# yangliu9527/Object_SLAM

Measured on AMD Instinct MI355X. Metric: frames/sec tracking+localBA, higher is better.
Workload: dtype f64

## Files before the change

### object_slam_amd/csrc/slam_driver.hip

```cpp
#include <atomic>
#include <chrono>
#include <map>
#include <memory>

#include "common.h"
#include "slam_map.h"
#include "slam_pool.h"

int oslam_slam_make_hip_ops(const oslam_slam_config_t* cfg, oslam_slam_ops_t* out);

namespace oslam_drv {

struct Vocab {
    uint64_t top[10][4], sub[10][10][4];
    Vocab() {
        uint64_t s = 0x853c49e6748fea9bULL;
        auto next = [&]() {
            const uint64_t old = s;
            s = old * 6364136223846793005ULL + 1442695040888963407ULL;
            const uint32_t x = (uint32_t)(((old >> 18u) ^ old) >> 27u), r = (uint32_t)(old >> 59u);
            return (x >> r) | (x << ((-r) & 31));
        };
        auto word = [&]() { const uint64_t hi = next(); const uint64_t lo = next(); return (hi << 32) | lo; };
        for (int i = 0; i < 10; i++)
// ... 237 lines not shown
    k.id = (int)s.map.kfs.size() - 1;
    k.frameId = f.id; k.stamp = f.stamp; k.N = f.N;
    if (!s.lazyKeys) k.keys.assign(f.keys.begin(), f.keys.begin() + f.N);
    k.keysUn.assign(f.keysUn.begin(), f.keysUn.begin() + f.N);
    k.oct.resize(f.N);
    for (int i = 0; i < f.N; i++) k.oct[i] = (uint8_t)f.keysUn[i].octave;
    if (!s.lazyDesc) k.desc.assign(f.desc.begin(), f.desc.begin() + (size_t)f.N * 32);
    k.uRight.assign(f.uRight.begin(), f.uRight.begin() + f.N);
    k.depth.assign(f.depth.begin(), f.depth.begin() + f.N);
    k.mp.assign(f.mp.begin(), f.mp.begin() + f.N);
    k.bowNode = f.bowNode;
    k.pose.set_keyframe(f.pose.Tcw);
    k.Tcp = eye4();
    s.counter.resize(s.map.kfs.size() + 8, 0);
    s.st[1]++;
    s.pendingKF.push_back(k.id);
    s.map.jr_new_kf(k.id);
    return k.id;
}

struct MpUpdate {
    struct Item { int seq, p; };
    std::vector<Item> items;
    std::vector<int> start;
    std::vector<uint8_t> odesc, outdesc;
    std::vector<int32_t> okey;
    std::vector<float> oOw, pos, owref, lsf, out5;
    std::vector<int> best;
    void clear() { items.clear(); }
    void add(int seq, int p) { items.push_back({seq, p}); }
    std::vector<int> dstart;
    std::vector<int32_t> ikey;
    struct Prof {
        std::atomic<long long> ns[4], calls{0}, pts{0}, obs{0};
        Prof() { for (auto& x : ns) x = 0; }
        ~Prof() {
            if (calls.load()) fprintf(stderr, "[mp_update prof] %lld calls, %lld points, %lld observations: count %.1f ms, pack %.1f ms, operator %.1f ms, scatter %.1f ms\n", calls.load(), pts.load(),
                                      obs.load(), ns[0] * 1e-6, ns[1] * 1e-6, ns[2] * 1e-6, ns[3] * 1e-6);
        }
    };
    static Prof* prof() { static Prof* p = getenv("OSLAM_MPU_PROF") ? new Prof : nullptr; static struct D { ~D() { delete prof(); } } d; return p; }
    bool pending = false, pDesc = false, pNormal = false;
    oslam_job_mp_update_t pjob;
    int run(Ctx& c, bool do_desc, bool do_normal) {
        const int rc = submit(c, do_desc, do_normal, false);
        return rc ? rc : finish(c);
    }
    int submit(Ctx& c, bool do_desc, bool do_normal, bool defer) {
        if (pending) { const int rc0 = finish(c); if (rc0) return rc0; }
        const int P = (int)items.size();
        if (P == 0) return OSLAM_OK;
        Prof* pf = prof();
        auto t0_ = std::chrono::steady_clock::now();
        auto lap_ = [&](int k) { if (pf) { auto t1_ = std::chrono::steady_clock::now(); pf->ns[k] += std::chrono::duration_cast<std::chrono::nanoseconds>(t1_ - t0_).count(); t0_ = t1_; } };
        start.assign(P + 1, 0); dstart.assign(P + 1, 0);
        const int chunk = 256, nchunks = (P + chunk - 1) / chunk;
        c.pool->parallel_for(nchunks, [&](int ch) {
            const int i0 = ch * chunk, i1 = std::min(P, i0 + chunk);
            for (int i = i0; i < i1; i++) {
                if (i + kPF < i1) prefetch_mp(&c.seq[items[i + kPF].seq]->map.mps[items[i + kPF].p]);
                if (i + kPF / 2 < i1) __builtin_prefetch(c.seq[items[i + kPF / 2].seq]->map.mps[items[i + kPF / 2].p].obs.data());
                const Map& m = c.seq[items[i].seq]->map;
                const MapPt& p = m.mps[items[i].p];
                int n = 0, nd = 0;
                if (!m.pBad[items[i].p]) { n = (int)p.obs.size(); for (auto& e : p.obs) nd += !m.kfs[e.first].bad; }
                start[i + 1] = n; dstart[i + 1] = nd;
            }
        });
        for (int i = 0; i < P; i++) { start[i + 1] += start[i]; dstart[i + 1] += dstart[i]; }
        lap_(0);
        const size_t total = (size_t)start[P], dtotal = (size_t)dstart[P];
        const bool split = dtotal != total;
        if (do_desc) c.badKFObs.fetch_add((long long)(total - dtotal), std::memory_order_relaxed);
        const bool keyed = c.ops.mp_update_keyed != nullptr && do_desc;
        if (!keyed) odesc.resize(do_desc ? std::max<size_t>(dtotal, 1) * 32 : 32);
        else okey.resize(std::max<size_t>(dtotal, 1) * 3);
        oOw.resize(std::max<size_t>(total, 1) * 3);
        pos.resize((size_t)P * 3); owref.resize((size_t)P * 3); lsf.resize(P);
        c.pool->parallel_for(nchunks, [&](int ch) {
            const int i0 = ch * chunk, i1 = std::min(P, i0 + chunk);
            for (int i = i0; i < i1; i++) {
                if (i + kPF < i1) prefetch_mp(&c.seq[items[i + kPF].seq]->map.mps[items[i + kPF].p]);
                if (i + kPF / 2 < i1) __builtin_prefetch(c.seq[items[i + kPF / 2].seq]->map.mps[items[i + kPF / 2].p].obs.data());
                if (do_normal && i + kPF / 2 < i1) __builtin_prefetch(c.seq[items[i + kPF / 2].seq]->map.mps[items[i + kPF / 2].p].okp.data());
                const Map& m = c.seq[items[i].seq]->map;
                const MapPt& p = m.mps[items[i].p];
                const int n = start[i + 1] - start[i];
                size_t at = (size_t)start[i], dat = (size_t)dstart[i];
                if (n > 0)
                    for (auto& e : p.obs) {
                        const KeyFrm& k = m.kfs[e.first];
                        if (do_desc && !k.bad) {
                            if (keyed) { okey[dat * 3] = items[i].seq; okey[dat * 3 + 1] = e.first; okey[dat * 3 + 2] = e.second; }
                            else memcpy(&odesc[dat * 32], &k.desc[(size_t)e.second * 32], 32);
                            dat++;
                        }
                        oOw[at * 3] = k.pose.Ow[0]; oOw[at * 3 + 1] = k.pose.Ow[1]; oOw[at * 3 + 2] = k.pose.Ow[2];
                        at++;
                    }
                for (int d = 0; d < 3; d++) pos[(size_t)i * 3 + d] = p.pos[d];
                float lf = 1.f;
                const float* ow = p.pos;
                if (n > 0 && p.refKF >= 0) {
                    const KeyFrm& rk = m.kfs[p.refKF];
                    ow = rk.pose.Ow;
                    for (size_t oi = 0; oi < p.obs.size(); oi++)
                        if (p.obs[oi].first == p.refKF) { lf = c.scale[p.okp[oi].octave]; break; }
                }
                for (int d = 0; d < 3; d++) owref[(size_t)i * 3 + d] = ow[d];
                lsf[i] = lf;
            }
        });
        lap_(1);
        best.resize(P); outdesc.resize((size_t)P * 32); out5.resize((size_t)P * 5);
        oslam_job_mp_update_t& j = pjob;
        j.P = P; j.obs_start = start.data(); j.obs_desc = keyed ? nullptr : odesc.data(); j.obs_Ow = oOw.data(); j.Pos = pos.data(); j.OwRef = owref.data();
        j.levelScaleFactor = lsf.data(); j.do_desc = do_desc; j.do_normal = do_normal; j.best_idx = best.data(); j.out_desc = outdesc.data(); j.out5 = out5.data();
        j.desc_start = split ? dstart.data() : nullptr;
        ikey.resize((size_t)P * 2);
        for (int i = 0; i < P; i++) { ikey[2 * (size_t)i] = items[i].seq; ikey[2 * (size_t)i + 1] = items[i].p; }
        j.items = ikey.data();
        const bool async = defer && keyed && c.ops.mp_update_keyed_async && c.ops.mp_update_collect;
        const int rc = async ? c.ops.mp_update_keyed_async(c.ops.ctx, &j, okey.data()) : keyed ? c.ops.mp_update_keyed(c.ops.ctx, &j, okey.data()) : c.ops.mp_update(c.ops.ctx, &j);
        if (rc) return rc;
        lap_(2);
        pending = true; pDesc = do_desc; pNormal = do_normal; pAsync = async;
        if (pf) { pf->calls++; pf->pts += P; pf->obs += (long long)total; }
        return OSLAM_OK;
    }
    bool pAsync = false;
    struct SpecStats { std::atomic<long long> upd{0}, changed{0}, changed_in_list{0}; ~SpecStats() { fprintf(stderr, "[fuse spec stats] per-round descriptor updates %lld, changed %lld, changed and in the current keyframe's candidate list %lld\n", upd.load(), changed.load(), changed_in_list.load()); } };
    int finish(Ctx& c) {
        static SpecStats* spec_stats = getenv("OSLAM_SLAM_SPEC_STATS") ? new SpecStats : nullptr;
        static struct SpecAtExit { ~SpecAtExit() { delete spec_stats; } } spec_at_exit;
        if (!pending) return OSLAM_OK;
        pending = false;
        if (pAsync) { const int rc = c.ops.mp_update_collect(c.ops.ctx); if (rc) return rc; }
        const bool do_desc = pDesc, do_normal = pNormal;
        const int P = (int)items.size();
        const int chunk = 256, nchunks = (P + chunk - 1) / chunk;
        Prof* pf = prof();
        auto t0_ = std::chrono::steady_clock::now();
        auto lap_ = [&](int k) { if (pf) { auto t1_ = std::chrono::steady_clock::now(); pf->ns[k] += std::chrono::duration_cast<std::chrono::nanoseconds>(t1_ - t0_).count(); t0_ = t1_; } };
        c.pool->parallel_for(nchunks, [&](int ch) {
            const int i0 = ch * chunk, i1 = std::min(P, i0 + chunk);
            for (int i = i0; i < i1; i++) {
                if (start[i + 1] == start[i]) continue;
                MapPt& p = c.seq[items[i].seq]->map.mps[items[i].p];
                if (spec_stats && do_desc && !do_normal && dstart[i + 1] > dstart[i]) {
                    spec_stats->upd++;
                    const Seq& sq = *c.seq[items[i].seq];
                    if (memcmp(p.desc, &outdesc[(size_t)i * 32], 32) != 0) { spec_stats->changed++; if (p.fuseListStamp == sq.curKF + 1) spec_stats->changed_in_list++; }
                }
                if (do_desc && dstart[i + 1] > dstart[i]) memcpy(p.desc, &outdesc[(size_t)i * 32], 32);
                if (do_normal) {
                    const float* o = &out5[(size_t)i * 5];
                    p.normal[0] = o[0]; p.normal[1] = o[1]; p.normal[2] = o[2]; p.maxD = o[3]; p.minD = o[4];
                }
                if (do_desc && do_normal) { p.updVer = p.obsVer; p.updStep = c.mapStep; }
            }
        });
        lap_(3);
        return OSLAM_OK;
    }
};

static void create_stereo_points(Ctx& c, Seq& s, Frame& f, int kf, bool all) {
// ... 2023 lines not shown
    TrackInput in(TrackInput::STEREO, left, gray_stride, on_device, timestamps, objs, mask_stride, Tcw_out, state_out);
    in.right = right;
    return track_checked(h, "oslam_slam_track_stereo_objects", in);
}

static void twc_rows(const M4& Tcw, float* o) {
    for (int r = 0; r < 3; r++) {
        for (int cc = 0; cc < 3; cc++) o[r * 4 + cc] = Tcw.m[cc * 4 + r];
        float s = Tcw.m[r] * Tcw.m[3];
        s += Tcw.m[4 + r] * Tcw.m[7];
        s += Tcw.m[8 + r] * Tcw.m[11];
        o[r * 4 + 3] = (float)((double)s * -1.0);
    }
}

int oslam_slam_trajectory(oslam_slam_t* h, int seq, int cap, double* stamps, float* Twc, int32_t* n_out) {
    if (!h || seq < 0 || seq >= h->c.S || !n_out) { oslam::set_error("oslam_slam_trajectory: bad argument"); return OSLAM_E_INVALID; }
    { const int rc_ = oslam_slam_finish(h); if (rc_) return rc_; }
    const Seq& s = *h->c.seq[seq];
    const Map& m = s.map;
    int n = 0;
    if (m.kfs.empty()) { *n_out = 0; return OSLAM_OK; }
    const M4 Two = m.kfs[0].pose.Twc;
    for (const RelPose& r : s.rel) {
        if (r.lost) continue;
        int k = r.refKF;
        M4 Trw = eye4();
        while (m.kfs[k].bad) { Trw = mul4(Trw, m.kfs[k].Tcp); k = m.kfs[k].parent; }
        Trw = mul4(mul4(Trw, m.kfs[k].pose.Tcw), Two);
        const M4 Tcw = mul4(r.Tcr, Trw);
        if (n < cap) {
            if (stamps) stamps[n] = r.stamp;
            if (Twc) twc_rows(Tcw, Twc + (size_t)n * 12);
        }
        n++;
    }
    *n_out = n;
    if (n > cap) { oslam::set_error("trajectory: cap %d < %d", cap, n); return OSLAM_E_CAPACITY; }
    return OSLAM_OK;
}

int oslam_slam_keyframe_trajectory(oslam_slam_t* h, int seq, int cap, double* stamps, float* Twc, int32_t* n_out) {
    if (!h || seq < 0 || seq >= h->c.S || !n_out) { oslam::set_error("oslam_slam_keyframe_trajectory: bad argument"); return OSLAM_E_INVALID; }
    { const int rc_ = oslam_slam_finish(h); if (rc_) return rc_; }
    const Map& m = h->c.seq[seq]->map;
    int n = 0;
    for (const KeyFrm& k : m.kfs) {
        if (k.bad) continue;
        if (n < cap) {
            if (stamps) stamps[n] = k.stamp;
            if (Twc)
                for (int r = 0; r < 3; r++) {
                    for (int cc = 0; cc < 3; cc++) Twc[(size_t)n * 12 + r * 4 + cc] = k.pose.Rwc[r * 3 + cc];
                    Twc[(size_t)n * 12 + r * 4 + 3] = k.pose.Ow[r];
                }
        }
        n++;
    }
    *n_out = n;
    if (n > cap) { oslam::set_error("keyframe trajectory: cap %d < %d", cap, n); return OSLAM_E_CAPACITY; }
    return OSLAM_OK;
}

int oslam_slam_stats(oslam_slam_t* h, int seq, int64_t out[16]) {
    if (!h || seq < 0 || seq >= h->c.S || !out) { oslam::set_error("oslam_slam_stats: bad argument"); return OSLAM_E_INVALID; }
    Seq& s = *h->c.seq[seq];
    memcpy(out, s.st, sizeof(s.st));
    out[2] = s.map.nKFsInMap; out[4] = s.map.nMPsInMap;
    out[15] = map_violations(s.map);
    return OSLAM_OK;
}

int oslam_slam_kernel_times(oslam_slam_t* h, int enable, double out[OSLAM_SLAM_KT_GROUPS * 3]) {
    if (!h) { oslam::set_error("oslam_slam_kernel_times: bad argument"); return OSLAM_E_INVALID; }
    if (!h->c.ops.kernel_times) { oslam::set_error("oslam_slam_kernel_times: this operator table has no device timing"); return OSLAM_E_INVALID; }
    return h->c.ops.kernel_times(h->c.ops.ctx, enable, out);
}

int oslam_slam_debug_point(oslam_slam_t* h, int seq, int id, uint8_t host[64], uint8_t resident[64], int32_t* bad) {
    if (!h || !host || !resident || !bad || seq < 0 || seq >= h->c.S) { oslam::set_error("oslam_slam_debug_point: bad argument"); return OSLAM_E_INVALID; }
    const Map& m = h->c.seq[seq]->map;
    if (id < 0 || id >= (int)m.mps.size()) { oslam::set_error("oslam_slam_debug_point: no such point"); return OSLAM_E_INVALID; }
    const MapPt& p = m.mps[id];
    static_assert(offsetof(MapPt, desc) == 32 && offsetof(MapPt, minD) == 24, "the first 64 bytes of MapPt are the resident record");
    memcpy(host, &p, 64);
    *bad = m.pBad[id] || p.obs.empty();
    if (!h->c.ops.point_record) { oslam::set_error("oslam_slam_debug_point: the operator table keeps no resident map points"); return OSLAM_E_INVALID; }
    return h->c.ops.point_record(h->c.ops.ctx, seq, id, resident);
}

int oslam_slam_bad_keyframe_observations(oslam_slam_t* h, int64_t* out) {
    if (!h || !out) { oslam::set_error("oslam_slam_bad_keyframe_observations: bad argument"); return OSLAM_E_INVALID; }
    *out = h->c.badKFObs.load();
    return OSLAM_OK;
}

int oslam_slam_local_map_reuse(oslam_slam_t* h, int64_t out[2]) {
    if (!h || !out) { oslam::set_error("oslam_slam_local_map_reuse: bad argument"); return OSLAM_E_INVALID; }
    out[0] = h->c.locReuse.load(); out[1] = h->c.locFrames.load();
    return OSLAM_OK;
}

int oslam_slam_struct_sizes(int32_t out[4]) {
    if (!out) return OSLAM_E_INVALID;
    out[0] = (int32_t)sizeof(oslam_slam_config_t); out[1] = (int32_t)sizeof(oslam_slam_ops_t); out[2] = (int32_t)sizeof(oslam_slam_objects_t); out[3] = (int32_t)sizeof(oslam_map_changes_t);
    return OSLAM_OK;
}

int oslam_slam_stage_cpu_seconds(oslam_slam_t* h, double out[16]) {
    if (!h || !out) { oslam::set_error("oslam_slam_stage_cpu_seconds: bad argument"); return OSLAM_E_INVALID; }
    memcpy(out, h->c.cpu, sizeof(h->c.cpu));
    return OSLAM_OK;
}

int oslam_slam_stage_seconds(oslam_slam_t* h, double out[16]) {
    if (!h || !out) { oslam::set_error("oslam_slam_stage_seconds: bad argument"); return OSLAM_E_INVALID; }
    memcpy(out, h->c.sec, sizeof(h->c.sec));
    return OSLAM_OK;
}

}
```

### object_slam_amd/csrc/slam_map.h

```cpp
#pragma once
#include <algorithm>
#include <cmath>
#include <cstdint>
#include <cstring>
#include <map>
#include <set>
#include <utility>
#include <vector>

#include "../../include/oslam_slam.h"

namespace oslam_drv {

typedef oslam_keypoint_t KP;

struct M4 { float m[16]; };
inline M4 eye4() { M4 r; memset(r.m, 0, sizeof(r.m)); r.m[0] = r.m[5] = r.m[10] = r.m[15] = 1.f; return r; }
inline M4 mul4(const M4& a, const M4& b) {
    M4 r;
    for (int i = 0; i < 4; i++)
        for (int j = 0; j < 4; j++) {
            float s = a.m[i * 4] * b.m[j];
            s += a.m[i * 4 + 1] * b.m[4 + j];
            s += a.m[i * 4 + 2] * b.m[8 + j];
            s += a.m[i * 4 + 3] * b.m[12 + j];
            r.m[i * 4 + j] = s;
        }
    return r;
}
inline float norm3(const float* v) {
    double s = 0;
    for (int k = 0; k < 3; k++) s += (double)v[k] * (double)v[k];
    return (float)std::sqrt(s);
}

struct PoseM {
    M4 Tcw, Twc;
    float Rwc[9], Ow[3];
    bool valid = false;
    void set_frame(const M4& T) {
        Tcw = T; valid = true;
        for (int r = 0; r < 3; r++)
            for (int c = 0; c < 3; c++) Rwc[r * 3 + c] = T.m[c * 4 + r];
        for (int r = 0; r < 3; r++) {
            double s = 0;
            for (int k = 0; k < 3; k++) s += (double)T.m[k * 4 + r] * (double)T.m[k * 4 + 3];
            Ow[r] = (float)(-1.0 * s);
        }
        fill_twc();
    }
    void set_keyframe(const M4& T) {
        Tcw = T; valid = true;
        for (int r = 0; r < 3; r++)
            for (int c = 0; c < 3; c++) Rwc[r * 3 + c] = T.m[c * 4 + r];
        for (int r = 0; r < 3; r++) {
            float s = Rwc[r * 3] * T.m[3];
            s += Rwc[r * 3 + 1] * T.m[7];
            s += Rwc[r * 3 + 2] * T.m[11];
            Ow[r] = (float)((double)s * -1.0);
        }
        fill_twc();
    }
    void fill_twc() {
        Twc = eye4();
        for (int r = 0; r < 3; r++) {
            for (int c = 0; c < 3; c++) Twc.m[r * 4 + c] = Rwc[r * 3 + c];
            Twc.m[r * 4 + 3] = Ow[r];
        }
    }
};

struct Frame {
    int id = -1;
    double stamp = 0;
    int N = 0;
    std::vector<KP> keys, keysUn;
    std::vector<uint8_t> desc;
    std::vector<float> uRight, depth;
    std::vector<int> mp;
    std::vector<uint8_t> outlier;
    std::vector<uint32_t> bowNode;
    PoseM pose;
    int refKF = -1;
    oslam_slam_frame_t view;
    struct Obj2D { int det = -1, track = -1, obj3d = -1; std::vector<int> kps; };
    std::vector<Obj2D> objs;
    std::vector<int> objOfKp;
    void alloc(int cap) {
        keys.resize(cap); keysUn.resize(cap); desc.resize((size_t)cap * 32); uRight.resize(cap); depth.resize(cap);
        mp.assign(cap, -1); outlier.assign(cap, 0);
        view.N = 0; view.keys = keys.data(); view.keysUn = keysUn.data(); view.desc = desc.data(); view.uRight = uRight.data(); view.depth = depth.data();
    }
    void begin(int id_, double stamp_) {
        id = id_; stamp = stamp_; N = view.N;
        std::fill(mp.begin(), mp.end(), -1);
        std::fill(outlier.begin(), outlier.end(), 0);
        bowNode.clear(); pose.valid = false; refKF = -1;
        objs.clear(); objOfKp.assign(N, -1);
    }
};

struct ObsKp { float x, y, ur; int octave; };

struct MapPt {
    float pos[3];
    float normal[3] = {0, 0, 0};
    float minD = 0, maxD = 0;
    uint8_t desc[32];
    int firstKF = 0, firstFrame = 0, refKF = -1;
    std::vector<std::pair<int, int>> obs;
    std::vector<ObsKp> okp;
    int trackRefForFrame = 0;
    int fuseListIdx = 0, fuseListStamp = 0;
    int obsVer = 0, updVer = -1, updStep = -1;
    int obs_index(int kf) const {
        for (size_t i = 0; i < obs.size(); i++) if (obs[i].first == kf) return obs[i].second;
        return -1;
    }
};

constexpr int kPF = 12;
inline void prefetch_mp(const MapPt* p) { __builtin_prefetch(p); __builtin_prefetch((const char*)p + 64); __builtin_prefetch((const char*)p + 128); }
template <class Ids>
inline void prefetch_ahead(const std::vector<MapPt>& mps, const Ids& ids, size_t i, size_t n) {
    if (i + kPF < n) { const int q = ids[i + kPF]; if (q >= 0) prefetch_mp(&mps[q]); }
}
template <class Ids>
inline void prefetch_obs_ahead(const std::vector<MapPt>& mps, const Ids& ids, size_t i, size_t n) {
    prefetch_ahead(mps, ids, i, n);
    if (i + kPF / 2 < n) { const int q = ids[i + kPF / 2]; if (q >= 0) __builtin_prefetch(mps[q].obs.data()); }
}

template <class Ids>
inline void prefetch_okp_ahead(const std::vector<MapPt>& mps, const Ids& ids, size_t i, size_t n) {
    prefetch_obs_ahead(mps, ids, i, n);
    if (i + kPF / 2 < n) { const int q = ids[i + kPF / 2]; if (q >= 0) __builtin_prefetch(mps[q].okp.data()); }
}

struct KeyFrm {
    int id = 0, frameId = 0;
    double stamp = 0;
    int N = 0;
    std::vector<KP> keys, keysUn;
    std::vector<uint8_t> desc, oct;
    std::vector<float> uRight, depth;
    std::vector<int> mp;
    std::vector<uint32_t> bowNode;
    PoseM pose;
    M4 Tcp;
    std::map<int, int> connW;
    std::vector<int> ordered, orderedW;
    int parent = -1;
    std::set<int> children;
    bool firstConnection = true, bad = false;
    int trackRefForFrame = 0, fuseTargetForKF = 0;
};

struct RelPose { M4 Tcr; int refKF; double stamp; bool lost; };

struct Map {
    std::vector<MapPt> mps;
    std::vector<KeyFrm> kfs;
    int nKFsInMap = 0, nMPsInMap = 0;
    int64_t nCulledKF = 0, nCulledMP = 0;

    std::vector<int> pNObs, pVisible, pFound, pLastSeen, pReplaced;
    std::vector<uint8_t> pBad;
    std::vector<uint64_t> pLvl;
    bool lvlOverflow = false;
    void lvl_add(int p, int oct) {
        if ((unsigned)oct >= 8u || ((pLvl[p] >> (8 * oct)) & 0xFFull) == 0xFFull) { lvlOverflow = true; return; }
        pLvl[p] += 1ull << (8 * oct);
    }
    void lvl_sub(int p, int oct) {
        if ((unsigned)oct >= 8u || ((pLvl[p] >> (8 * oct)) & 0xFFull) == 0ull) { lvlOverflow = true; return; }
        pLvl[p] -= 1ull << (8 * oct);
    }
    int lvl_count_le(int p, int oct) const {
        const uint64_t h = oct >= 7 ? pLvl[p] : (pLvl[p] & ((1ull << (8 * (oct + 1))) - 1ull));
        uint64_t s2 = (h & 0x00FF00FF00FF00FFull) + ((h >> 8) & 0x00FF00FF00FF00FFull);
        s2 = (s2 & 0x0000FFFF0000FFFFull) + ((s2 >> 16) & 0x0000FFFF0000FFFFull);
        return (int)((s2 & 0xFFFFFFFFull) + (s2 >> 32));
    }
    enum { JR_KFMP = 1, JR_KFMP_BULK = 2, JR_OKF_SET = 3, JR_OKF_CLR = 4, JR_PT = 5, JR_RESET = 6 };
    bool jrOn = false, jrReset = false;
    std::vector<std::pair<int, int>> jrCells;
    std::vector<uint32_t> jrOkf;
    std::vector<int> jrPts, jrNewKFs;
    std::vector<uint8_t> jrPtMark;
    bool jr_pending() const { return jrReset || !jrCells.empty() || !jrOkf.empty() || !jrPts.empty() || !jrNewKFs.empty(); }
    void jr_kfmp(int kf, int idx, int) { if (jrOn) jrCells.push_back(std::make_pair(kf, idx)); }
    void jr_okf(int op, int kf, int idx, int p) { if (jrOn) { jrOkf.push_back((uint32_t)kf); jrOkf.push_back((uint32_t)idx | (op == JR_OKF_SET ? 0x80000000u : 0u)); jrOkf.push_back((uint32_t)p); } }
    void jr_pt(int p) {
        if (!jrOn) return;
        if (jrPtMark.size() <= (size_t)p) jrPtMark.resize((size_t)p + 1 + jrPtMark.size() / 2, 0);
        if (!jrPtMark[p]) { jrPtMark[p] = 1; jrPts.push_back(p); }
    }
    void jr_new_kf(int kf) { if (jrOn) jrNewKFs.push_back(kf); }
    struct JrScratch { std::vector<oslam_map_new_kf_t> kfs; std::vector<uint32_t> good, pts; std::vector<int32_t> cells; std::vector<uint32_t> events; };
    void journal_changes(int slot, float thDepth, JrScratch& sc, oslam_map_changes_t& ch) {
        ch.slot = slot; ch.reset = jrReset ? 1 : 0; jrReset = false;
        sc.kfs.clear(); sc.good.clear();
        size_t gw = 0;
        for (int kf : jrNewKFs) gw += (kfs[kf].mp.size() + 31) / 32;
        sc.good.resize(gw);
        gw = 0;
        for (int kf : jrNewKFs) {
            const KeyFrm& k = kfs[kf];
            const size_t N = k.mp.size(), nw = (N + 31) / 32;
            for (size_t wI = 0; wI < nw; wI++) {
                uint32_t bits = 0;
                for (size_t i = wI * 32; i < std::min(N, wI * 32 + 32); i++) bits |= (uint32_t)(!(k.depth[i] > thDepth || k.depth[i] < 0)) << (i & 31);
                sc.good[gw + wI] = bits;
            }
            oslam_map_new_kf_t e; e.kf = kf; e.N = (int32_t)N; e.mp = k.mp.data(); e.good = nullptr;
            sc.kfs.push_back(e);
            gw += nw;
        }
        gw = 0;
        for (auto& e : sc.kfs) { e.good = sc.good.data() + gw; gw += ((size_t)e.N + 31) / 32; }
        sc.cells.resize(jrCells.size() * 3);
        for (size_t i = 0; i < jrCells.size(); i++) { sc.cells[3 * i] = jrCells[i].first; sc.cells[3 * i + 1] = jrCells[i].second; sc.cells[3 * i + 2] = kfs[jrCells[i].first].mp[jrCells[i].second]; }
        sc.events.swap(jrOkf);
        sc.pts.resize(jrPts.size() * 5);
        for (size_t i = 0; i < jrPts.size(); i++) {
            const int p = jrPts[i];
            jrPtMark[p] = 0;
            sc.pts[5 * i] = (uint32_t)p; sc.pts[5 * i + 1] = (uint32_t)pNObs[p]; sc.pts[5 * i + 2] = (uint32_t)pBad[p];
            sc.pts[5 * i + 3] = (uint32_t)(pLvl[p] & 0xFFFFFFFFull); sc.pts[5 * i + 4] = (uint32_t)(pLvl[p] >> 32);
        }
        ch.n_new = (int32_t)sc.kfs.size(); ch.new_kfs = sc.kfs.data();
        ch.n_cells = (int32_t)jrCells.size(); ch.cells = sc.cells.data();
        ch.n_events = (int32_t)(sc.events.size() / 3); ch.events = sc.events.data();
        ch.n_points = (int32_t)jrPts.size(); ch.points = sc.pts.data();
        jrNewKFs.clear(); jrCells.clear(); jrOkf.clear(); jrPts.clear();
    }
    void set_kf_mp(int kf, int idx, int p) { kfs[kf].mp[idx] = p; jr_kfmp(kf, idx, p); }

    int new_point(const float x[3], int refKF, int refFrame) {
        MapPt p;
        p.pos[0] = x[0]; p.pos[1] = x[1]; p.pos[2] = x[2];
        memset(p.desc, 0, 32);
        p.firstKF = refKF; p.firstFrame = refFrame; p.refKF = refKF;
        mps.push_back(p);
        pNObs.push_back(0); pVisible.push_back(1); pFound.push_back(1);
        pLastSeen.push_back(0); pReplaced.push_back(-1); pBad.push_back(0); pLvl.push_back(0);
        return (int)mps.size() - 1;
    }
    void add_observation(int p, int kf, int idx) {
        MapPt& m = mps[p];
        size_t at = 0;
        while (at < m.obs.size() && m.obs[at].first < kf) at++;
        if (at < m.obs.size() && m.obs[at].first == kf) return;
        const KeyFrm& k = kfs[kf];
        const ObsKp o = {k.keysUn[idx].x, k.keysUn[idx].y, k.uRight[idx], k.keysUn[idx].octave};
        m.obs.insert(m.obs.begin() + at, std::make_pair(kf, idx));
        m.okp.insert(m.okp.begin() + at, o);
        lvl_add(p, o.octave);
        pNObs[p] += o.ur >= 0 ? 2 : 1;
        m.obsVer++;
        jr_okf(JR_OKF_SET, kf, idx, p); jr_pt(p);
    }
    void set_bad_point(int p) {
        MapPt& m = mps[p];
        if (!pBad[p]) { nMPsInMap--; nCulledMP++; }
        pBad[p] = 1;
        std::vector<std::pair<int, int>> o;
        o.swap(m.obs);
        std::vector<ObsKp>().swap(m.okp);
        pLvl[p] = 0;
        for (auto& e : o) { set_kf_mp(e.first, e.second, -1); jr_okf(JR_OKF_CLR, e.first, e.second, p); }
        jr_pt(p);
    }
    void erase_observation(int p, int kf) {
        MapPt& m = mps[p];
        bool bad = false;
        for (size_t i = 0; i < m.obs.size(); i++)
            if (m.obs[i].first == kf) {
                pNObs[p] -= m.okp[i].ur >= 0 ? 2 : 1;
                jr_okf(JR_OKF_CLR, kf, m.obs[i].second, p);
                m.obs.erase(m.obs.begin() + i);
                lvl_sub(p, m.okp[i].octave);
                m.okp.erase(m.okp.begin() + i);
                m.obsVer++;
                if (m.refKF == kf && !m.obs.empty()) m.refKF = m.obs.front().first;
                if (pNObs[p] <= 2) bad = true;
                jr_pt(p);
                break;
            }
        if (bad) set_bad_point(p);
    }
    bool replace_point(int p, int by) {
        if (p == by) return false;
        MapPt& m = mps[p];
        std::vector<std::pair<int, int>> o;
        o.swap(m.obs);
        std::vector<ObsKp>().swap(m.okp);
        pLvl[p] = 0;
        if (!pBad[p]) { nMPsInMap--; }
        pBad[p] = 1;
        pReplaced[p] = by;
        const int nvisible = pVisible[p], nfound = pFound[p];
        for (auto& e : o) {
            jr_okf(JR_OKF_CLR, e.first, e.second, p);
            if (mps[by].obs_index(e.first) < 0) {
                set_kf_mp(e.first, e.second, by);
                add_observation(by, e.first, e.second);
            } else {
                set_kf_mp(e.first, e.second, -1);
            }
        }
        jr_pt(p);
        pFound[by] += nfound;
        pVisible[by] += nvisible;
        return true;
    }

    void update_best_covisibles(int k) {
        KeyFrm& f = kfs[k];
        static thread_local std::vector<std::pair<int, int>> v;
        v.clear();
        for (auto& e : f.connW) v.push_back(std::make_pair(e.second, e.first));
        std::sort(v.begin(), v.end());
        f.ordered.clear(); f.orderedW.clear();
        for (size_t i = v.size(); i-- > 0;) { f.ordered.push_back(v[i].second); f.orderedW.push_back(v[i].first); }
    }
    void add_connection(int k, int other, int w) {
        KeyFrm& f = kfs[k];
        auto it = f.connW.find(other);
        if (it == f.connW.end()) f.connW[other] = w;
        else if (it->second != w) it->second = w;
        else return;
        update_best_covisibles(k);
    }
    void erase_connection(int k, int other) {
        if (kfs[k].connW.erase(other)) update_best_covisibles(k);
    }
    struct IntSpan {
        const int* b; const int* e;
        const int* begin() const { return b; }
        const int* end() const { return e; }
        size_t size() const { return (size_t)(e - b); }
    };
    IntSpan best_covisibles(int k, int n) const {
        const KeyFrm& f = kfs[k];
        const size_t m = std::min<size_t>(f.ordered.size(), (size_t)std::max(n, 0));
        return IntSpan{f.ordered.data(), f.ordered.data() + m};
    }
    int weight(int k, int other) const {
        auto it = kfs[k].connW.find(other);
        return it == kfs[k].connW.end() ? 0 : it->second;
    }
    void update_connections(int k, std::vector<int>& counter ) {
        KeyFrm& f = kfs[k];
        static thread_local std::vector<int> touched;
        touched.clear();
        for (int i = 0; i < f.N; i++) {
            prefetch_obs_ahead(mps, f.mp, i, f.N);
            const int p = f.mp[i];
            if (p < 0 || pBad[p]) continue;
            for (auto& e : mps[p].obs) {
                if (e.first == k) continue;
                if (counter[e.first]++ == 0) touched.push_back(e.first);
            }
        }
        if (touched.empty()) return;
        std::sort(touched.begin(), touched.end());
        int nmax = 0, kmax = -1;
        const int th = 15;
        static thread_local std::vector<std::pair<int, int>> v2;
        std::vector<std::pair<int, int>>& v = v2;
        v.clear();
        for (int o : touched) {
            const int c = counter[o];
            if (c > nmax) { nmax = c; kmax = o; }
            if (c >= th) { v.push_back(std::make_pair(c, o)); add_connection(o, k, c); }
        }
        if (v.empty()) { v.push_back(std::make_pair(nmax, kmax)); add_connection(kmax, k, nmax); }
        std::sort(v.begin(), v.end());
        f.connW.clear();
        for (int o : touched) { f.connW[o] = counter[o]; counter[o] = 0; }
        f.ordered.clear(); f.orderedW.clear();
        for (size_t i = v.size(); i-- > 0;) { f.ordered.push_back(v[i].second); f.orderedW.push_back(v[i].first); }
        if (f.firstConnection && f.id != 0) {
            f.parent = f.ordered.front();
            kfs[f.parent].children.insert(k);
            f.firstConnection = false;
        }
    }
    int tracked_map_points(int k, int minObs) const {
        const KeyFrm& f = kfs[k];
        int n = 0;
        for (int i = 0; i < f.N; i++) {
            const int p = f.mp[i];
// ... 44 lines not shown
```

Baseline: 46560.

## Move map points and observation lists into a per-sequence slab arena

Map points now live in a chunked table backed by a per-sequence arena built on hugepage-advised mmap slabs. Each point's observation and keypoint lists, which were two std::vectors, become one arena block holding both arrays. MapPt is repacked to 128 bytes with the per-frame fields in the first cache line. The aim is to cut malloc traffic, pointer chasing and TLB misses during tracking and local BA. In exchange it adds custom allocator complexity, and the table can no longer be copied or grown as a contiguous vector.

```diff
diff --git a/object_slam_amd/csrc/seq_arena.h b/object_slam_amd/csrc/seq_arena.h
--- /dev/null
+++ b/object_slam_amd/csrc/seq_arena.h
@@ -0,0 +1,221 @@
+#pragma once
+#include <cstddef>
+#include <cstdint>
+#include <cstdlib>
+#include <cstring>
+#include <mutex>
+#include <new>
+#include <type_traits>
+
+#ifndef OSLAM_ARENA_PASSTHROUGH
+#include <sys/mman.h>
+#endif
+
+#ifndef OSLAM_ARENA_CHUNK_KB
+#define OSLAM_ARENA_CHUNK_KB 16
+#endif
+
+namespace oslam_drv {
+
+constexpr size_t kArenaChunk = (size_t)OSLAM_ARENA_CHUNK_KB << 10;
+constexpr size_t kArenaSlab = (size_t)64 << 20;
+constexpr size_t kArenaHuge = (size_t)2 << 20;
+constexpr size_t kArenaChunkHead = 64;
+
+struct ArenaChunk { ArenaChunk* next; };
+
+struct SlabPoolStats { size_t slabs, chunks_carved, chunks_free, madvise_failed; bool hugepages; };
+
+#ifndef OSLAM_ARENA_PASSTHROUGH
+class SlabPool {
+public:
+    static SlabPool& instance() { static SlabPool p; return p; }
+    ArenaChunk* take() {
+        std::lock_guard<std::mutex> g(mu_);
+        if (free_) { ArenaChunk* c = free_; free_ = c->next; nFree_--; return c; }
+        if (cur_ == end_) {
+            char* raw = (char*)mmap(nullptr, kArenaSlab + kArenaHuge, PROT_READ | PROT_WRITE, MAP_PRIVATE | MAP_ANONYMOUS, -1, 0);
+            if (raw == (char*)MAP_FAILED) throw std::bad_alloc();
+            char* al = (char*)(((uintptr_t)raw + kArenaHuge - 1) & ~(uintptr_t)(kArenaHuge - 1));
+            if (al > raw) munmap(raw, (size_t)(al - raw));
+            if (al + kArenaSlab < raw + kArenaSlab + kArenaHuge) munmap(al + kArenaSlab, (size_t)(raw + kArenaHuge - al));
+            if (huge_ && madvise(al, kArenaSlab, MADV_HUGEPAGE) != 0) nMadvFail_++;
+            cur_ = al; end_ = al + kArenaSlab; nSlabs_++;
+        }
+        ArenaChunk* c = (ArenaChunk*)cur_;
+        cur_ += kArenaChunk; nCarved_++;
+        return c;
+    }
+    void give(ArenaChunk* head, ArenaChunk* tail, size_t n) {
+        std::lock_guard<std::mutex> g(mu_);
+        tail->next = free_; free_ = head; nFree_ += n;
+    }
+    SlabPoolStats stats() {
+        std::lock_guard<std::mutex> g(mu_);
+        return SlabPoolStats{nSlabs_, nCarved_, nFree_, nMadvFail_, huge_};
+    }
+private:
+    SlabPool() { const char* e = getenv("OSLAM_MAP_HUGEPAGES"); huge_ = !(e && e[0] == '0'); }
+    std::mutex mu_;
+    ArenaChunk* free_ = nullptr;
+    char *cur_ = nullptr, *end_ = nullptr;
+    size_t nSlabs_ = 0, nCarved_ = 0, nFree_ = 0, nMadvFail_ = 0;
+    bool huge_ = true;
+};
+#endif
+
+class SeqArena {
+public:
+    static constexpr int kClasses = 24;
+    static size_t class_units(int c) { return c == 0 ? 1 : (c & 1) ? (size_t)1 << ((c + 1) / 2) : (size_t)3 << (c / 2 - 1); }
+    static size_t class_bytes(int c) { return class_units(c) << 4; }
+    static int class_of(size_t bytes) {
+        const size_t u = (bytes + 15) >> 4;
+        if (u <= 1) return 0;
+        const int p = 63 - __builtin_clzll((unsigned long long)u);
+        if (u == (size_t)1 << p) return 2 * p - 1;
+        if (u <= (size_t)3 << (p - 1)) return 2 * p;
+        return 2 * p + 1;
+    }
+    static constexpr size_t kMaxSmall = kArenaChunk / 2;
+
+    SeqArena() = default;
+    SeqArena(const SeqArena&) = delete;
+    SeqArena& operator=(const SeqArena&) = delete;
+    SeqArena(SeqArena&& o) noexcept { steal(o); }
+    SeqArena& operator=(SeqArena&& o) noexcept { if (this != &o) { release(); steal(o); } return *this; }
+    ~SeqArena() { release(); }
+
+    void* alloc(size_t bytes) {
+#ifndef OSLAM_ARENA_PASSTHROUGH
+        if (bytes <= kMaxSmall) {
+            const int c = class_of(bytes);
+            if (free_[c]) { void* p = free_[c]; free_[c] = *(void**)p; return p; }
+            const size_t sz = class_bytes(c);
+            if (void* p = bump(sz)) return p;
+            for (int c2 = c + 1; c2 < kClasses; c2++)
+                if (free_[c2]) {
+                    char* b = (char*)free_[c2]; free_[c2] = *(void**)b;
+                    recycle(b + sz, b + class_bytes(c2));
+                    return b;
+                }
+            if (cur_) recycle(cur_, end_);
+            ArenaChunk* ch = SlabPool::instance().take();
+            ch->next = chunks_; chunks_ = ch; nChunks_++;
+            if (!lastChunk_) lastChunk_ = ch;
+            cur_ = (char*)ch + kArenaChunkHead; end_ = (char*)ch + kArenaChunk;
+            return bump(sz);
+        }
+#endif
+        return tracked_alloc(bytes);
+    }
+    void dealloc(void* p, size_t bytes) {
+        if (!p) return;
+#ifndef OSLAM_ARENA_PASSTHROUGH
+        if (bytes <= kMaxSmall) { const int c = class_of(bytes); *(void**)p = free_[c]; free_[c] = p; return; }
+#endif
+        (void)bytes;
+        tracked_free(p);
+    }
+    void release() {
+        while (big_) tracked_free((char*)big_ + sizeof(Big));
+#ifndef OSLAM_ARENA_PASSTHROUGH
+        if (chunks_) SlabPool::instance().give(chunks_, lastChunk_, nChunks_);
+        chunks_ = lastChunk_ = nullptr; nChunks_ = 0; cur_ = end_ = nullptr;
+        memset(free_, 0, sizeof(free_));
+#endif
+    }
+    size_t chunks_held() const { return nChunks_; }
+
+private:
+    struct alignas(64) Big { Big *prev, *next; };
+    void* tracked_alloc(size_t bytes) {
+        void* raw = nullptr;
+        if (posix_memalign(&raw, 64, sizeof(Big) + bytes) != 0) throw std::bad_alloc();
+        Big* b = (Big*)raw;
+        b->prev = nullptr; b->next = big_;
+        if (big_) big_->prev = b;
+        big_ = b;
+        return (char*)b + sizeof(Big);
+    }
+    void tracked_free(void* p) {
+        Big* b = (Big*)((char*)p - sizeof(Big));
+        if (b->prev) b->prev->next = b->next; else big_ = b->next;
+        if (b->next) b->next->prev = b->prev;
+        free(b);
+    }
+    void steal(SeqArena& o) {
+        big_ = o.big_; o.big_ = nullptr;
+        chunks_ = o.chunks_; lastChunk_ = o.lastChunk_; nChunks_ = o.nChunks_; cur_ = o.cur_; end_ = o.end_;
+        memcpy(free_, o.free_, sizeof(free_));
+        o.chunks_ = o.lastChunk_ = nullptr; o.nChunks_ = 0; o.cur_ = o.end_ = nullptr;
+        memset(o.free_, 0, sizeof(o.free_));
+    }
+#ifndef OSLAM_ARENA_PASSTHROUGH
+    void* bump(size_t sz) {
+        if (!cur_) return nullptr;
+        char* p = cur_;
+        if (sz >= 1024) p = (char*)(((uintptr_t)p + 63) & ~(uintptr_t)63);
+        if (p + sz > end_) return nullptr;
+        if (p != cur_) recycle(cur_, p);
+        cur_ = p + sz;
+        return p;
+    }
+    void recycle(char* b, char* e) {
+        while (e - b >= 16) {
+            size_t rem = (size_t)(e - b);
+            if (rem > kMaxSmall) rem = kMaxSmall;
+            int c = class_of(rem);
+            if (class_bytes(c) > rem) c--;
+            const size_t mis = (uintptr_t)b & 63;
+            if (class_bytes(c) >= 1024 && mis) c = class_of(64 - mis);
+            *(void**)b = free_[c]; free_[c] = b;
+            b += class_bytes(c);
+        }
+    }
+#endif
+    Big* big_ = nullptr;
+    ArenaChunk *chunks_ = nullptr, *lastChunk_ = nullptr;
+    size_t nChunks_ = 0;
+    char *cur_ = nullptr, *end_ = nullptr;
+    void* free_[kClasses] = {};
+};
+
+template <class T, int K>
+struct ChunkVec {
+    static_assert(std::is_trivially_copyable<T>::value && std::is_trivially_destructible<T>::value, "ChunkVec holds plain data");
+    static constexpr size_t kMask = ((size_t)1 << K) - 1;
+    T** blk = nullptr;
+    uint32_t nblk = 0, capblk = 0;
+    size_t n = 0;
+    ChunkVec() = default;
+    ChunkVec(const ChunkVec&) = delete;
+    ChunkVec& operator=(const ChunkVec&) = delete;
+    ChunkVec(ChunkVec&& o) noexcept : blk(o.blk), nblk(o.nblk), capblk(o.capblk), n(o.n) { o.blk = nullptr; o.nblk = o.capblk = 0; o.n = 0; }
+    ChunkVec& operator=(ChunkVec&& o) noexcept {
+        if (this != &o) { blk = o.blk; nblk = o.nblk; capblk = o.capblk; n = o.n; o.blk = nullptr; o.nblk = o.capblk = 0; o.n = 0; }
+        return *this;
+    }
+    T& operator[](size_t i) { return blk[i >> K][i & kMask]; }
+    const T& operator[](size_t i) const { return blk[i >> K][i & kMask]; }
+    size_t size() const { return n; }
+    bool empty() const { return n == 0; }
+    T& back() { return (*this)[n - 1]; }
+    const T& back() const { return (*this)[n - 1]; }
+    void push_back(SeqArena& a, const T& v) {
+        if ((n >> K) == nblk) {
+            if (nblk == capblk) {
+                const uint32_t nc = capblk ? capblk * 2 : 4;
+                T** nb = (T**)a.alloc(sizeof(T*) * nc);
+                if (nblk) memcpy(nb, blk, sizeof(T*) * nblk);
+                a.dealloc(blk, sizeof(T*) * capblk);
+                blk = nb; capblk = nc;
+            }
+            blk[nblk++] = (T*)a.alloc(sizeof(T) << K);
+        }
+        memcpy(&blk[n >> K][n & kMask], &v, sizeof(T));
+        n++;
+    }
+};
+
+}
diff --git a/object_slam_amd/csrc/slam_driver.hip b/object_slam_amd/csrc/slam_driver.hip
--- a/object_slam_amd/csrc/slam_driver.hip
+++ b/object_slam_amd/csrc/slam_driver.hip
@@ -343,7 +343,6 @@
             for (int i = i0; i < i1; i++) {
                 if (i + kPF < i1) prefetch_mp(&c.seq[items[i + kPF].seq]->map.mps[items[i + kPF].p]);
                 if (i + kPF / 2 < i1) __builtin_prefetch(c.seq[items[i + kPF / 2].seq]->map.mps[items[i + kPF / 2].p].obs.data());
-                if (do_normal && i + kPF / 2 < i1) __builtin_prefetch(c.seq[items[i + kPF / 2].seq]->map.mps[items[i + kPF / 2].p].okp.data());
                 const Map& m = c.seq[items[i].seq]->map;
                 const MapPt& p = m.mps[items[i].p];
                 const int n = start[i + 1] - start[i];
@@ -2533,8 +2532,7 @@
     const Map& m = h->c.seq[seq]->map;
     if (id < 0 || id >= (int)m.mps.size()) { oslam::set_error("oslam_slam_debug_point: no such point"); return OSLAM_E_INVALID; }
     const MapPt& p = m.mps[id];
-    static_assert(offsetof(MapPt, desc) == 32 && offsetof(MapPt, minD) == 24, "the first 64 bytes of MapPt are the resident record");
-    memcpy(host, &p, 64);
+    memcpy(host, p.pos, 12); memcpy(host + 12, p.normal, 12); memcpy(host + 24, &p.minD, 4); memcpy(host + 28, &p.maxD, 4); memcpy(host + 32, p.desc, 32);
     *bad = m.pBad[id] || p.obs.empty();
     if (!h->c.ops.point_record) { oslam::set_error("oslam_slam_debug_point: the operator table keeps no resident map points"); return OSLAM_E_INVALID; }
     return h->c.ops.point_record(h->c.ops.ctx, seq, id, resident);
diff --git a/object_slam_amd/csrc/slam_map.h b/object_slam_amd/csrc/slam_map.h
--- a/object_slam_amd/csrc/slam_map.h
+++ b/object_slam_amd/csrc/slam_map.h
@@ -9,6 +9,7 @@
 #include <vector>
 
 #include "../../include/oslam_slam.h"
+#include "seq_arena.h"
 
 namespace oslam_drv {
 
@@ -101,40 +102,67 @@
 };
 
 struct ObsKp { float x, y, ur; int octave; };
-
-struct MapPt {
+typedef std::pair<int, int> Obs;
+
+struct ObsListRaw { char* blk; uint32_t n, cap; };
+struct ObsView {
+    char* blk; uint32_t n, cap;
+    size_t size() const { return n; }
+    bool empty() const { return n == 0; }
+    const Obs* data() const { return (const Obs*)blk; }
+    const Obs* begin() const { return data(); }
+    const Obs* end() const { return data() + n; }
+    const Obs& operator[](size_t i) const { return data()[i]; }
+    const Obs& front() const { return data()[0]; }
+};
+struct OkpView {
+    char* blk; uint32_t n, cap;
+    size_t size() const { return n; }
+    bool empty() const { return n == 0; }
+    const ObsKp* data() const { return (const ObsKp*)(blk + (size_t)cap * sizeof(Obs)); }
+    const ObsKp* begin() const { return data(); }
+    const ObsKp* end() const { return data() + n; }
+    const ObsKp& operator[](size_t i) const { return data()[i]; }
+    const ObsKp& front() const { return data()[0]; }
+};
+constexpr size_t obs_block_bytes(uint32_t cap) { return (size_t)cap * (sizeof(Obs) + sizeof(ObsKp)); }
+
+struct alignas(64) MapPt {
+    union { ObsListRaw lst = {nullptr, 0, 0}; ObsView obs; OkpView okp; };
     float pos[3];
     float normal[3] = {0, 0, 0};
     float minD = 0, maxD = 0;
-    uint8_t desc[32];
-    int firstKF = 0, firstFrame = 0, refKF = -1;
-    std::vector<std::pair<int, int>> obs;
-    std::vector<ObsKp> okp;
+    int refKF = -1;
     int trackRefForFrame = 0;
     int fuseListIdx = 0, fuseListStamp = 0;
+    uint8_t desc[32];
+    int firstKF = 0, firstFrame = 0;
     int obsVer = 0, updVer = -1, updStep = -1;
     int obs_index(int kf) const {
         for (size_t i = 0; i < obs.size(); i++) if (obs[i].first == kf) return obs[i].second;
         return -1;
     }
 };
+static_assert(sizeof(MapPt) == 128 && offsetof(MapPt, desc) == 64, "MapPt: two cache lines, the per-frame fields in the first");
+
+typedef ChunkVec<MapPt, 6> PtTable;
+static_assert((sizeof(MapPt) << 6) <= SeqArena::kMaxSmall, "a block of the point table is an arena block");
+template <class T> using PtArray = ChunkVec<T, 8>;
 
 constexpr int kPF = 12;
-inline void prefetch_mp(const MapPt* p) { __builtin_prefetch(p); __builtin_prefetch((const char*)p + 64); __builtin_prefetch((const char*)p + 128); }
+inline void prefetch_mp(const MapPt* p) { __builtin_prefetch(p); __builtin_prefetch((const char*)p + 64); }
 template <class Ids>
-inline void prefetch_ahead(const std::vector<MapPt>& mps, const Ids& ids, size_t i, size_t n) {
+inline void prefetch_ahead(const PtTable& mps, const Ids& ids, size_t i, size_t n) {
     if (i + kPF < n) { const int q = ids[i + kPF]; if (q >= 0) prefetch_mp(&mps[q]); }
 }
 template <class Ids>
-inline void prefetch_obs_ahead(const std::vector<MapPt>& mps, const Ids& ids, size_t i, size_t n) {
+inline void prefetch_obs_ahead(const PtTable& mps, const Ids& ids, size_t i, size_t n) {
     prefetch_ahead(mps, ids, i, n);
     if (i + kPF / 2 < n) { const int q = ids[i + kPF / 2]; if (q >= 0) __builtin_prefetch(mps[q].obs.data()); }
 }
-
 template <class Ids>
-inline void prefetch_okp_ahead(const std::vector<MapPt>& mps, const Ids& ids, size_t i, size_t n) {
+inline void prefetch_okp_ahead(const PtTable& mps, const Ids& ids, size_t i, size_t n) {
     prefetch_obs_ahead(mps, ids, i, n);
-    if (i + kPF / 2 < n) { const int q = ids[i + kPF / 2]; if (q >= 0) __builtin_prefetch(mps[q].okp.data()); }
 }
 
 struct KeyFrm {
@@ -159,14 +187,18 @@
 struct RelPose { M4 Tcr; int refKF; double stamp; bool lost; };
 
 struct Map {
-    std::vector<MapPt> mps;
+    SeqArena arena;
+    PtTable mps;
     std::vector<KeyFrm> kfs;
+    Map() = default;
+    Map(Map&&) = default;
+    Map& operator=(Map&&) = default;
     int nKFsInMap = 0, nMPsInMap = 0;
     int64_t nCulledKF = 0, nCulledMP = 0;
 
-    std::vector<int> pNObs, pVisible, pFound, pLastSeen, pReplaced;
-    std::vector<uint8_t> pBad;
-    std::vector<uint64_t> pLvl;
+    PtArray<int> pNObs, pVisible, pFound, pLastSeen, pReplaced;
+    PtArray<uint8_t> pBad;
+    PtArray<uint64_t> pLvl;
     bool lvlOverflow = false;
     void lvl_add(int p, int oct) {
         if ((unsigned)oct >= 8u || ((pLvl[p] >> (8 * oct)) & 0xFFull) == 0xFFull) { lvlOverflow = true; return; }
@@ -242,11 +274,44 @@
         p.pos[0] = x[0]; p.pos[1] = x[1]; p.pos[2] = x[2];
         memset(p.desc, 0, 32);
         p.firstKF = refKF; p.firstFrame = refFrame; p.refKF = refKF;
-        mps.push_back(p);
-        pNObs.push_back(0); pVisible.push_back(1); pFound.push_back(1);
-        pLastSeen.push_back(0); pReplaced.push_back(-1); pBad.push_back(0); pLvl.push_back(0);
+        mps.push_back(arena, p);
+        pNObs.push_back(arena, 0); pVisible.push_back(arena, 1); pFound.push_back(arena, 1);
+        pLastSeen.push_back(arena, 0); pReplaced.push_back(arena, -1); pBad.push_back(arena, 0); pLvl.push_back(arena, 0);
         return (int)mps.size() - 1;
     }
+    void list_insert(MapPt& m, size_t at, const Obs& e, const ObsKp& o) {
+        ObsListRaw& l = m.lst;
+        const size_t n = l.n;
+        if (l.n == l.cap) {
+            const uint32_t ncap = l.cap ? l.cap * 2 : 2;
+            char* nb = (char*)arena.alloc(obs_block_bytes(ncap));
+            Obs* no = (Obs*)nb; ObsKp* nk = (ObsKp*)(nb + (size_t)ncap * sizeof(Obs));
+            if (n) {
+                const Obs* oo = m.obs.data(); const ObsKp* ok = m.okp.data();
+                memcpy((void*)no, (const void*)oo, at * sizeof(Obs)); memcpy((void*)(no + at + 1), (const void*)(oo + at), (n - at) * sizeof(Obs));
+                memcpy(nk, ok, at * sizeof(ObsKp)); memcpy(nk + at + 1, ok + at, (n - at) * sizeof(ObsKp));
+            }
+            arena.dealloc(l.blk, obs_block_bytes(l.cap));
+            l.blk = nb; l.cap = ncap;
+        } else {
+            Obs* oo = (Obs*)l.blk; ObsKp* ok = (ObsKp*)(l.blk + (size_t)l.cap * sizeof(Obs));
+            memmove((void*)(oo + at + 1), (const void*)(oo + at), (n - at) * sizeof(Obs));
+            memmove(ok + at + 1, ok + at, (n - at) * sizeof(ObsKp));
+        }
+        ((Obs*)l.blk)[at] = e;
+        ((ObsKp*)(l.blk + (size_t)l.cap * sizeof(Obs)))[at] = o;
+        l.n++;
+    }
+    void list_erase(MapPt& m, size_t at) {
+        ObsListRaw& l = m.lst;
+        Obs* oo = (Obs*)l.blk; ObsKp* ok = (ObsKp*)(l.blk + (size_t)l.cap * sizeof(Obs));
+        memmove((void*)(oo + at), (const void*)(oo + at + 1), (l.n - at - 1) * sizeof(Obs));
+        memmove(ok + at, ok + at + 1, (l.n - at - 1) * sizeof(ObsKp));
+        l.n--;
+    }
+    ObsListRaw list_detach(MapPt& m) { const ObsListRaw l = m.lst; m.lst = ObsListRaw{nullptr, 0, 0}; return l; }
+    void list_drop(const ObsListRaw& l) { arena.dealloc(l.blk, obs_block_bytes(l.cap)); }
+
     void add_observation(int p, int kf, int idx) {
         MapPt& m = mps[p];
         size_t at = 0;
@@ -254,8 +319,7 @@
         if (at < m.obs.size() && m.obs[at].first == kf) return;
         const KeyFrm& k = kfs[kf];
         const ObsKp o = {k.keysUn[idx].x, k.keysUn[idx].y, k.uRight[idx], k.keysUn[idx].octave};
-        m.obs.insert(m.obs.begin() + at, std::make_pair(kf, idx));
-        m.okp.insert(m.okp.begin() + at, o);
+        list_insert(m, at, std::make_pair(kf, idx), o);
         lvl_add(p, o.octave);
         pNObs[p] += o.ur >= 0 ? 2 : 1;
         m.obsVer++;
@@ -265,11 +329,11 @@
         MapPt& m = mps[p];
         if (!pBad[p]) { nMPsInMap--; nCulledMP++; }
         pBad[p] = 1;
-        std::vector<std::pair<int, int>> o;
-        o.swap(m.obs);
-        std::vector<ObsKp>().swap(m.okp);
+        const ObsListRaw o = list_detach(m);
         pLvl[p] = 0;
-        for (auto& e : o) { set_kf_mp(e.first, e.second, -1); jr_okf(JR_OKF_CLR, e.first, e.second, p); }
+        const Obs* oe = (const Obs*)o.blk;
+        for (uint32_t i = 0; i < o.n; i++) { set_kf_mp(oe[i].first, oe[i].second, -1); jr_okf(JR_OKF_CLR, oe[i].first, oe[i].second, p); }
+        list_drop(o);
         jr_pt(p);
     }
     void erase_observation(int p, int kf) {
@@ -277,11 +341,11 @@
         bool bad = false;
         for (size_t i = 0; i < m.obs.size(); i++)
             if (m.obs[i].first == kf) {
-                pNObs[p] -= m.okp[i].ur >= 0 ? 2 : 1;
+                const ObsKp o = m.okp[i];
+                pNObs[p] -= o.ur >= 0 ? 2 : 1;
                 jr_okf(JR_OKF_CLR, kf, m.obs[i].second, p);
-                m.obs.erase(m.obs.begin() + i);
-                lvl_sub(p, m.okp[i].octave);
-                m.okp.erase(m.okp.begin() + i);
+                list_erase(m, i);
+                lvl_sub(p, o.octave);
                 m.obsVer++;
                 if (m.refKF == kf && !m.obs.empty()) m.refKF = m.obs.front().first;
                 if (pNObs[p] <= 2) bad = true;
@@ -293,15 +357,15 @@
     bool replace_point(int p, int by) {
         if (p == by) return false;
         MapPt& m = mps[p];
-        std::vector<std::pair<int, int>> o;
-        o.swap(m.obs);
-        std::vector<ObsKp>().swap(m.okp);
+        const ObsListRaw o = list_detach(m);
         pLvl[p] = 0;
         if (!pBad[p]) { nMPsInMap--; }
         pBad[p] = 1;
         pReplaced[p] = by;
         const int nvisible = pVisible[p], nfound = pFound[p];
-        for (auto& e : o) {
+        const Obs* oe = (const Obs*)o.blk;
+        for (uint32_t i = 0; i < o.n; i++) {
+            const Obs e = oe[i];
             jr_okf(JR_OKF_CLR, e.first, e.second, p);
             if (mps[by].obs_index(e.first) < 0) {
                 set_kf_mp(e.first, e.second, by);
@@ -310,6 +374,7 @@
                 set_kf_mp(e.first, e.second, -1);
             }
         }
+        list_drop(o);
         jr_pt(p);
         pFound[by] += nfound;
         pVisible[by] += nvisible;
```

Result: faster. 52190, median of 6 (+12.1%).
